# 1812598631/Amos-slam

Measured on AMD Instinct MI355X. Metric: front-end frames/sec (ORB extract+match+mask) at 640x480, higher is better.
Workload: dtype u8 (ORB, gate, matcher) + fp32 (mask network); 1 GPU; configs[2]: 640x480 L8 N1000 full front-end: YOLACT-R50 fp32 mask + ORB detect + gate + describe + match; lanes_per_gpu=2, frames_per_launch=64, width=640, height=480, n_features=1000, n_levels=8, ini_th_fast=20, min_th_fast=7, match=frame k vs k-1, N x N best-2, synthetic_stream_seed=stream = rank, frame k seeded 1000*rank+k (amos-slam_amd/synth.py), parallelism=frames sharded 1 ways, one process per GPU, no data-path collective

## Files before the change

amos-slam_amd/__init__.py:

```python
import ctypes as C
import os

import numpy as np

_HERE = os.path.dirname(os.path.abspath(__file__))
LIB_PATH = os.environ.get("AMOS_FRONTEND_LIB", os.path.join(_HERE, "csrc", "libamos_frontend.so"))

KP_DTYPE = np.dtype([("x", "<f4"), ("y", "<f4"), ("size", "<f4"), ("angle", "<f4"),
                     ("response", "<f4"), ("octave", "<i4"), ("class_id", "<i4")])
BEST2_DTYPE = np.dtype([("best_idx", "<i4"), ("best_dist", "<i4"), ("second_idx", "<i4"),
                        ("second_dist", "<i4")])

TH_HIGH, TH_LOW, HISTO_LENGTH = 100, 50, 30

EXPORTS = [
    "amos_last_error", "amos_device_count", "amos_current_device", "amos_build_variant", "amos_orb_tables_host", "amos_orb_geometry_probe", "amos_orb_create", "amos_orb_destroy", "amos_orb_tables",
    "amos_orb_level_sizes", "amos_orb_detect", "amos_orb_level_count", "amos_orb_level_keypoints",
    "amos_orb_set_level_keypoints", "amos_orb_level_layout", "amos_orb_fetch_levels", "amos_orb_store_levels", "amos_orb_gate", "amos_orb_closed_mask", "amos_orb_describe",
    "amos_orb_extract", "amos_orb_level_image", "amos_orb_pyramid_images", "amos_orb_blurred_image", "amos_orb_level_candidates",
    "amos_orb_extract_batch_device", "amos_orb_detect_batch_device", "amos_orb_gate_batch_device",
    "amos_orb_describe_batch_device", "amos_orb_extract_batch_device_color", "amos_frame_rgbd_glue_batch_device", "amos_frame_undistort_batch_device", "amos_frame_image_bounds", "amos_frame_grid_build_batch_device", "amos_match_window_best2_batch_device",
    "amos_orb_batch_results_device", "amos_orb_batch_fetch", "amos_orb_sync",
    "amos_orb_stream", "amos_orb_timing_enable", "amos_orb_timing_collect", "amos_match_create", "amos_match_destroy", "amos_match_sync", "amos_match_stream",
    "amos_match_distances", "amos_match_list_distances", "amos_match_list_best2", "amos_match_bruteforce_best2",
    "amos_match_bruteforce_best2_batch_device", "amos_match_set_bruteforce_kernel", "amos_slic_center_count", "amos_slic_create", "amos_slic_destroy", "amos_slic_stream",
    "amos_slic_run", "amos_slic_batch_device", "amos_cluster_kmeans_batch_device", "amos_cluster_kmeans", "amos_cluster_bgr2lab_batch_device", "amos_flow_check_device", "amos_flow_epipolar_device", "amos_flow_scene_flow_device", "amos_flow_fundamental_score_device", "amos_flow_pnp_score_device", "amos_lk_create", "amos_lk_destroy", "amos_lk_stream", "amos_lk_levels", "amos_lk_track_device", "amos_mask_pre_create", "amos_mask_pre_destroy", "amos_mask_pre_stream", "amos_mask_preprocess_batch_device", "amos_mask_bias_act_device", "amos_mask_bias_relu_maxpool_device", "amos_mask_stem_weight_floats", "amos_mask_stem_weights_device", "amos_mask_stem_device", "amos_mask_conv1x1_supported", "amos_mask_conv1x1_device", "amos_mask_conv_supported", "amos_mask_conv_device", "amos_mask_conv_workspace_bytes", "amos_mask_conv_ws_device", "amos_mask_conv_tile_mode", "amos_mask_conv_kernel_name", "amos_corners_create", "amos_corners_destroy", "amos_corners_stream", "amos_corners_good_features_device", "amos_corners_candidate_count", "amos_corners_subpix_device", "amos_fmat_create", "amos_fmat_destroy", "amos_fmat_stream", "amos_fmat_ransac_device", "amos_fmat_scene_flow_pair_device", "amos_fmat_ransac", "amos_mask_winograd_supported", "amos_mask_winograd_weight_floats", "amos_mask_winograd_weights_device", "amos_mask_winograd_conv_device", "amos_mask_winograd24_weight_floats", "amos_mask_winograd24_weights_device", "amos_mask_winograd24_conv_device", "amos_mask_winograd24_conv_layout_device", "amos_mask_winograd24_persistent_mode", "amos_mask_winograd24_narrow_mode", "amos_mask_bilinear_nhwc_device", "amos_mask_bilinear_nhwc_act_device", "amos_mask_bilinear_x2_mode", "amos_mask_nms_column_max_device", "amos_mask_class_scores_device", "amos_mask_person_mask_device", "amos_mask_head_outputs_device", "amos_mask_head_outputs_scores_device", "amos_mask_person_masks_scores_device", "amos_mask_topk_rows_device", "amos_mask_topk_rows_sparse_device", "amos_mask_post_workspace_bytes", "amos_mask_person_masks_device", "amos_orb_detect_color_with_mask_pre_batch_device",
]


class AmosError(RuntimeError):
    pass


class OrbParams(C.Structure):
    _fields_ = [("n_features", C.c_int32), ("scale_factor", C.c_float), ("n_levels", C.c_int32),
                ("ini_th_fast", C.c_int32), ("min_th_fast", C.c_int32)]


_lib = None


def lib():
    global _lib
    if _lib is None:
        if not os.path.exists(LIB_PATH):
            raise AmosError(f"{LIB_PATH} is missing: build it with `make -C amos-slam_amd/csrc` "
                            "(or __graft_entry__.build()); there is no CPU fallback")
        try:
            import torch
        except ImportError:
            pass
        L = C.CDLL(LIB_PATH)
        L.amos_last_error.restype = C.c_char_p
        L.amos_build_variant.restype = C.c_char_p
        variant = L.amos_build_variant().decode()
        if variant != "default" and os.environ.get("AMOS_ALLOW_EXPERIMENT_BUILD") != "1":
            raise AmosError(f"{LIB_PATH} is an experiment build ({variant}): its results are wrong; unset AMOS_FRONTEND_LIB "
                            "or set AMOS_ALLOW_EXPERIMENT_BUILD=1 for a timing run")
        L.amos_orb_stream.restype = C.c_void_p
# ... 427 lines not shown

def mask_winograd24_conv_layout(stream_ptr, x_ptr, u_ptr, bias_ptr, residual_ptr, y_ptr, batch, h, w, cin, cout, relu, in_blocked, out_blocked):
    _check(lib().amos_mask_winograd24_conv_layout_device(C.c_void_p(stream_ptr), C.c_void_p(x_ptr), C.c_void_p(u_ptr), C.c_void_p(bias_ptr),
                                                         C.c_void_p(residual_ptr), C.c_void_p(y_ptr), C.c_int(batch), C.c_int(h), C.c_int(w), C.c_int(cin),
                                                         C.c_int(cout), C.c_int(int(relu)), C.c_int(int(in_blocked)), C.c_int(int(out_blocked))),
           "amos_mask_winograd24_conv_layout_device")


def mask_winograd24_persistent_mode(mode=-2):
    return int(lib().amos_mask_winograd24_persistent_mode(C.c_int(mode)))


def mask_winograd24_narrow_mode(mode=-2):
    return int(lib().amos_mask_winograd24_narrow_mode(C.c_int(mode)))


def mask_conv_tile_mode(mode=-2):
    return int(lib().amos_mask_conv_tile_mode(C.c_int(mode)))


def mask_conv_kernel_name(batch, in_h, in_w, cin, cout, kh, kw, stride, pad):
    buf = C.create_string_buffer(96)
    _check(lib().amos_mask_conv_kernel_name(C.c_int(batch), C.c_int(in_h), C.c_int(in_w), C.c_int(cin), C.c_int(cout), C.c_int(kh), C.c_int(kw),
                                            C.c_int(stride), C.c_int(pad), buf, C.c_int(96)), "amos_mask_conv_kernel_name")
    return buf.value.decode()


def mask_conv(stream_ptr, x_ptr, w_ptr, bias_ptr, residual_ptr, y_ptr, batch, in_h, in_w, cin, cout, kh, kw, stride, pad, relu):
    _check(lib().amos_mask_conv_device(C.c_void_p(stream_ptr), C.c_void_p(x_ptr), C.c_void_p(w_ptr), C.c_void_p(bias_ptr), C.c_void_p(residual_ptr),
                                       C.c_void_p(y_ptr), C.c_int(batch), C.c_int(in_h), C.c_int(in_w), C.c_int(cin), C.c_int(cout), C.c_int(kh), C.c_int(kw),
                                       C.c_int(stride), C.c_int(pad), C.c_int(int(relu))), "amos_mask_conv_device")


def mask_conv_workspace_bytes(batch, in_h, in_w, cin, cout, kh, kw, stride, pad):
    fn = lib().amos_mask_conv_workspace_bytes
    fn.restype = C.c_size_t
    return int(fn(C.c_int(batch), C.c_int(in_h), C.c_int(in_w), C.c_int(cin), C.c_int(cout), C.c_int(kh), C.c_int(kw), C.c_int(stride), C.c_int(pad)))


def mask_conv_ws(stream_ptr, x_ptr, w_ptr, bias_ptr, residual_ptr, y_ptr, batch, in_h, in_w, cin, cout, kh, kw, stride, pad, relu, workspace_ptr, workspace_bytes):
    _check(lib().amos_mask_conv_ws_device(C.c_void_p(stream_ptr), C.c_void_p(x_ptr), C.c_void_p(w_ptr), C.c_void_p(bias_ptr), C.c_void_p(residual_ptr),
                                          C.c_void_p(y_ptr), C.c_int(batch), C.c_int(in_h), C.c_int(in_w), C.c_int(cin), C.c_int(cout), C.c_int(kh), C.c_int(kw),
                                          C.c_int(stride), C.c_int(pad), C.c_int(int(relu)), C.c_void_p(workspace_ptr), C.c_size_t(workspace_bytes)),
           "amos_mask_conv_ws_device")


def mask_bilinear_nhwc(stream_ptr, x_ptr, y_ptr, n, in_h, in_w, out_h, out_w, channels, scale_h, scale_w, relu=False):
    _check(lib().amos_mask_bilinear_nhwc_act_device(C.c_void_p(stream_ptr), C.c_void_p(x_ptr), C.c_void_p(y_ptr), C.c_int(n), C.c_int(in_h), C.c_int(in_w),
                                                    C.c_int(out_h), C.c_int(out_w), C.c_int(channels), C.c_float(scale_h), C.c_float(scale_w), C.c_int(int(relu))),
           "amos_mask_bilinear_nhwc_act_device")


def mask_class_scores(stream_ptr, conf_ptr, scores_ptr, batch, n_priors, n_classes_with_background, threshold):
    _check(lib().amos_mask_class_scores_device(C.c_void_p(stream_ptr), C.c_void_p(conf_ptr), C.c_void_p(scores_ptr), C.c_int(batch), C.c_int(n_priors),
                                               C.c_int(n_classes_with_background), C.c_float(threshold)), "amos_mask_class_scores_device")


def mask_person_mask(stream_ptr, masks_ptr, flags_ptr, out_ptr, batch, n_det, mask_h, mask_w, out_h, out_w):
    _check(lib().amos_mask_person_mask_device(C.c_void_p(stream_ptr), C.c_void_p(masks_ptr), C.c_void_p(flags_ptr), C.c_void_p(out_ptr), C.c_int(batch),
                                              C.c_int(n_det), C.c_int(mask_h), C.c_int(mask_w), C.c_int(out_h), C.c_int(out_w)), "amos_mask_person_mask_device")


def mask_head_outputs(stream_ptr, raw_ptr, bias_ptr, loc_ptr, conf_ptr, coef_ptr, batch, cells, channels_padded, anchors, n_classes_with_background, mask_dim,
                      n_priors_total, prior_offset):
    _check(lib().amos_mask_head_outputs_device(C.c_void_p(stream_ptr), C.c_void_p(raw_ptr), C.c_void_p(bias_ptr), C.c_void_p(loc_ptr), C.c_void_p(conf_ptr),
                                               C.c_void_p(coef_ptr), C.c_int(batch), C.c_int(cells), C.c_int(channels_padded), C.c_int(anchors),
# ... 262 lines not shown
```

amos-slam_amd/csrc/amos_conv1x1.hip:

```cpp
#include <hip/hip_runtime.h>
#include <stdint.h>
#include <stdio.h>
#include <stdlib.h>

#include <algorithm>

#include "../../include/amos_frontend.h"
#include "amos_common.h"

namespace amos {

constexpr int kGemmBK = 32;
constexpr int kGemmPitch = kGemmBK + 4;

typedef float f32x16 __attribute__((ext_vector_type(16)));

__device__ __attribute__((aligned(16))) const float g_conv_zeros[4] = {0.f, 0.f, 0.f, 0.f};

struct ConvGemmArgs {
    const float *x, *w, *bias, *res;
    float *y;
    int M, N, K;
    int outW, outHW, inW, inH;
    int stride, relu, mTiles, nTiles;
    int kh, kw, pad;
    int splits, stagesPerSplit;
    float *partial;
    unsigned *counters;
};

template <int WM, int WN, int TI, bool kTaps>
__global__ __launch_bounds__(256) __attribute__((amdgpu_waves_per_eu(1, 2))) void k_conv_gemm(const ConvGemmArgs a)
{
    constexpr int BM = 32 * TI * WM, BN = 64 * WN;
    constexpr int XP = BM / 32, WP = BN / 32;
    constexpr int kStage = (BM + BN) * kGemmPitch;
    static_assert(2 * kStage >= BM * BN, "the epilogue stages the output tile in the same LDS");
    __shared__ __align__(16) float smem[2 * kStage];
    float(*Xs)[kStage] = reinterpret_cast<float(*)[kStage]>(smem);
    float(*Ws)[kStage] = reinterpret_cast<float(*)[kStage]>(smem + BM * kGemmPitch);
    const int xcd = blockIdx.x & 7, seq = blockIdx.x >> 3;
    const int nt = a.splits > 1 ? (int)blockIdx.x % a.nTiles : seq % a.nTiles;
    const int mt = a.splits > 1 ? (int)blockIdx.x / a.nTiles : (seq / a.nTiles) * 8 + xcd;
    if (mt >= a.mTiles) return;
    const int t = threadIdx.x, lane = t & 63, wave = t >> 6;
    const int wm = wave / WN, wn = wave % WN;
    const int pc = t & 7, pr = t >> 3;
    const float *xsrc[XP];
    int iy0[XP], ix0[XP];
#pragma unroll
    for (int i = 0; i < XP; i++) {
        const int m = min(mt * BM + pr + 32 * i, a.M - 1);
        iy0[i] = ix0[i] = 0;
        if (!kTaps && a.stride == 1) {
            xsrc[i] = a.x + (size_t)m * a.K + 4 * pc;
        } else {
            const int b = m / a.outHW, rem = m - b * a.outHW, oy = rem / a.outW, ox = rem - oy * a.outW;
            iy0[i] = oy * a.stride - a.pad;
            ix0[i] = ox * a.stride - a.pad;
            xsrc[i] = a.x + (((ptrdiff_t)b * a.inH + iy0[i]) * a.inW + ix0[i]) * a.K + 4 * pc;
        }
    }
    const int kcPerTap = a.K / kGemmBK, wRow = a.K * a.kh * a.kw;
    const float *wsrc[WP];
#pragma unroll
    for (int j = 0; j < WP; j++) wsrc[j] = a.w + (size_t)(nt * BN + pr + 32 * j) * wRow + 4 * pc;
    static_assert(XP == 4 && (WP == 2 || WP == 4), "the staging registers below are named one by one");
    float4 x0, x1, x2, x3, w0, w1, w2 = {}, w3 = {};
    const int stagesAll = (a.K / kGemmBK) * a.kh * a.kw;
    const int sBegin = a.splits > 1 ? (int)blockIdx.y * a.stagesPerSplit : 0;
    const int sEnd = a.splits > 1 ? min(sBegin + a.stagesPerSplit, stagesAll) : stagesAll;
    int fKc = 0, fDy = 0, fDx = 0;
    if (kTaps && sBegin > 0) {
        const int kcPerTap0 = a.K / kGemmBK, tap = sBegin / kcPerTap0;
        fKc = sBegin - tap * kcPerTap0;
        fDy = tap / a.kw;
        fDx = tap - fDy * a.kw;
    }
    typedef float f32x4 __attribute__((ext_vector_type(4)));
    typedef const __attribute__((address_space(1))) f32x4 *GlobalF4;
// ... 60 lines not shown
    _Pragma("unroll") for (int q = 0; q < (n); q++) {                                     \
        __builtin_amdgcn_sched_group_barrier(0x008, 1, 0);                                \
        __builtin_amdgcn_sched_group_barrier(mask, 1, 0);                                 \
    }
    constexpr int kFragReads = TI + 2, kMfmas = 8 * TI;
#define AMOS_GEMM_STAGE(s, buf, kStash, kFetch, kNext)                                    \
    {                                                                                     \
        AMOS_GEMM_LDFRAG(fa1, fb1, buf, 1);                                               \
        AMOS_GEMM_MFMAS(fa0, fb0);                                                        \
        AMOS_GEMM_INTERLEAVE(0x100, kFragReads);                                          \
        __builtin_amdgcn_sched_group_barrier(0x008, kMfmas, 0);                           \
        __builtin_amdgcn_sched_barrier(0);                                                \
        AMOS_GEMM_LDFRAG(fa0, fb0, buf, 2);                                               \
        if (kStash) AMOS_GEMM_STASH((buf) ^ 1);                                           \
        AMOS_GEMM_MFMAS(fa1, fb1);                                                        \
        AMOS_GEMM_INTERLEAVE(0x100, kFragReads);                                          \
        AMOS_GEMM_INTERLEAVE(0x200, XP + WP);                                             \
        __builtin_amdgcn_sched_group_barrier(0x008, kMfmas, 0);                           \
        __builtin_amdgcn_sched_barrier(0);                                                \
        AMOS_GEMM_LDFRAG(fa1, fb1, buf, 3);                                               \
        if (kFetch) AMOS_GEMM_FETCH((s) + 2);                                             \
        AMOS_GEMM_MFMAS(fa0, fb0);                                                        \
        AMOS_GEMM_INTERLEAVE(0x100, kFragReads);                                          \
        AMOS_GEMM_INTERLEAVE(0x020, XP + WP);                                             \
        __builtin_amdgcn_sched_group_barrier(0x008, kMfmas, 0);                           \
        __builtin_amdgcn_sched_barrier(0);                                                \
        __syncthreads();                                                                  \
        if (kNext) AMOS_GEMM_LDFRAG(fa0, fb0, (buf) ^ 1, 0);                              \
        AMOS_GEMM_MFMAS(fa1, fb1);                                                        \
        AMOS_GEMM_INTERLEAVE(0x100, kFragReads);                                          \
        __builtin_amdgcn_sched_group_barrier(0x008, kMfmas, 0);                           \
        __builtin_amdgcn_sched_barrier(0);                                                \
    }
    f32x16 acc[TI][2];
#pragma unroll
    for (int i = 0; i < TI; i++)
#pragma unroll
        for (int j = 0; j < 2; j++)
#pragma unroll
            for (int r = 0; r < 16; r++) acc[i][j][r] = 0.f;
    const int xoff = (wm * 32 * TI + (lane & 31)) * kGemmPitch + 4 * (lane >> 5);
    const int woff = (wn * 64 + (lane & 31)) * kGemmPitch + 4 * (lane >> 5);
    const int stages = sEnd - sBegin;
    AMOS_GEMM_FETCH(sBegin);
    AMOS_GEMM_STASH(0);
    if (stages > 1) AMOS_GEMM_FETCH(sBegin + 1);
    __syncthreads();
    AMOS_GEMM_LDFRAG(fa0, fb0, 0, 0);
    int s = 0;
    for (; s + 2 < stages; s++) {
        const int buf = s & 1;
        AMOS_GEMM_STAGE(sBegin + s, buf, true, true, true);
    }
    if (s + 1 < stages) {
        const int buf = s & 1;
        AMOS_GEMM_STAGE(sBegin + s, buf, true, false, true);
        s++;
    }
    {
        const int buf = s & 1;
        AMOS_GEMM_STAGE(sBegin + s, buf, false, false, false);
    }
#undef AMOS_GEMM_FETCH
#undef AMOS_GEMM_TAPSRC
#undef AMOS_GEMM_STASH
#undef AMOS_GEMM_LDFRAG
#undef AMOS_GEMM_MFMAS
#undef AMOS_GEMM_INTERLEAVE
#undef AMOS_GEMM_STAGE
    __syncthreads();
#pragma unroll
    for (int i = 0; i < TI; i++)
#pragma unroll
        for (int j = 0; j < 2; j++)
#pragma unroll
            for (int r = 0; r < 16; r++)
                smem[(wm * 32 * TI + i * 32 + (r & 3) + 8 * (r >> 2) + 4 * (lane >> 5)) * BN + wn * 64 + j * 32 + (lane & 31)] = acc[i][j][r];
    __syncthreads();
    constexpr int kCols = BN / 4, kRowsPerPass = 256 / kCols, kPasses = BM / kRowsPerPass;
    const int oc = t % kCols, orow = t / kCols;
    const int n0 = nt * BN + 4 * oc;
    if (a.splits > 1) {
        __shared__ unsigned sArrived;
        const int tile = mt * a.nTiles + nt, nTilesAll = a.mTiles * a.nTiles;
        const unsigned xcc = __builtin_amdgcn_s_getreg((3 << 11) | 20) & 15u;
        const bool home = xcc == (blockIdx.x & 7u);
        float *mine = a.partial + ((size_t)blockIdx.y * nTilesAll + tile) * (BM * BN);
#pragma unroll
        for (int q = 0; q < kPasses; q++) {
            const int e = (q * kRowsPerPass + orow) * BN + 4 * oc;
            *reinterpret_cast<float4 *>(mine + e) = *reinterpret_cast<const float4 *>(&smem[e]);
        }
        if (home) asm volatile("s_waitcnt vmcnt(0)" ::: "memory");
        else __threadfence();
        __syncthreads();
        if (t == 0) sArrived = atomicAdd(&a.counters[tile], home ? 1u : 0x10001u);
        __syncthreads();
        const unsigned arrived = sArrived;
        if ((arrived & 0xffffu) != (unsigned)(a.splits - 1)) return;
        if (!home || (arrived >> 16) != 0) __threadfence();
#pragma unroll
        for (int q = 0; q < kPasses; q++) {
            const int e = (q * kRowsPerPass + orow) * BN + 4 * oc;
            float4 sum = {0.f, 0.f, 0.f, 0.f};
            for (int sp = 0; sp < a.splits; sp++) {
                typedef float f32x4v __attribute__((ext_vector_type(4)));
                const f32x4v v = *reinterpret_cast<const volatile f32x4v *>(a.partial + ((size_t)sp * nTilesAll + tile) * (BM * BN) + e);
                sum.x = sp ? sum.x + v.x : v.x; sum.y = sp ? sum.y + v.y : v.y; sum.z = sp ? sum.z + v.z : v.z; sum.w = sp ? sum.w + v.w : v.w;
            }
            *reinterpret_cast<float4 *>(&smem[e]) = sum;
        }
        if (t == 0) atomicExch(&a.counters[tile], 0u);
    }
    const float4 bv = a.bias ? *reinterpret_cast<const float4 *>(a.bias + n0) : float4{0.f, 0.f, 0.f, 0.f};
    constexpr int kBatch = 8;
#pragma unroll
    for (int p0 = 0; p0 < kPasses; p0 += kBatch) {
        float4 rv[kBatch];
#pragma unroll
        for (int q = 0; q < kBatch; q++) {
            const int m = mt * BM + (p0 + q) * kRowsPerPass + orow;
            rv[q] = (a.res && m < a.M) ? *reinterpret_cast<const float4 *>(a.res + (size_t)m * a.N + n0) : float4{0.f, 0.f, 0.f, 0.f};
        }
#pragma unroll
        for (int q = 0; q < kBatch; q++) {
            const int row = (p0 + q) * kRowsPerPass + orow, m = mt * BM + row;
            if (m >= a.M) continue;
            float4 v = *reinterpret_cast<const float4 *>(&smem[row * BN + 4 * oc]);
            v.x = (v.x + bv.x) + rv[q].x; v.y = (v.y + bv.y) + rv[q].y; v.z = (v.z + bv.z) + rv[q].z; v.w = (v.w + bv.w) + rv[q].w;
            if (a.relu) { v.x = fmaxf(v.x, 0.f); v.y = fmaxf(v.y, 0.f); v.z = fmaxf(v.z, 0.f); v.w = fmaxf(v.w, 0.f); }
            *reinterpret_cast<float4 *>(a.y + (size_t)m * a.N + n0) = v;
        }
    }
}

}

using namespace amos;

static int g_gemm_tile_mode = -2;

static int gemm_tile_mode()
{
    if (g_gemm_tile_mode == -2) {
        const char *env = getenv("AMOS_GEMM_NARROW");
        g_gemm_tile_mode = env && (env[0] == '0' || env[0] == '1') ? env[0] - '0' : -1;
    }
    return g_gemm_tile_mode;
}

static bool gemm_wide_tiles(long long M, int cout)
{
    const int mode = gemm_tile_mode();
    const long long wideGroups = ((M + 127) / 128) * (cout / 128);
    const bool narrow = mode >= 0 ? mode == 1 : wideGroups < 1024;
    return cout % 128 == 0 && !narrow;
}

extern "C" {

int amos_mask_conv_tile_mode(int mode)
{
    const int before = gemm_tile_mode();
// ... 44 lines not shown
    return (size_t)kSplitCounterBytes + (size_t)splits * tiles * 128 * (wide ? 128 : 64) * sizeof(float);
}

int amos_mask_conv_device(void *stream, const float *d_x, const float *d_w, const float *d_bias, const float *d_residual, float *d_y, int batch,
                          int in_h, int in_w, int cin, int cout, int kh, int kw, int stride, int pad, int relu)
{
    return amos_mask_conv_ws_device(stream, d_x, d_w, d_bias, d_residual, d_y, batch, in_h, in_w, cin, cout, kh, kw, stride, pad, relu, nullptr, 0);
}

int amos_mask_conv_ws_device(void *stream, const float *d_x, const float *d_w, const float *d_bias, const float *d_residual, float *d_y, int batch,
                             int in_h, int in_w, int cin, int cout, int kh, int kw, int stride, int pad, int relu, void *d_workspace, size_t workspace_bytes)
{
    if (!d_x || !d_w || !d_y || batch < 1 || in_h < 1 || in_w < 1 || amos_mask_conv_supported(cin, cout, kh, kw, stride, pad) != AMOS_OK ||
        in_h + 2 * pad < kh || in_w + 2 * pad < kw || ((uintptr_t)d_x | (uintptr_t)d_w | (uintptr_t)d_y | (uintptr_t)d_bias | (uintptr_t)d_residual) % 16 != 0) {
        set_error("amos_mask_conv_device: invalid argument (cin %% 32 == 0, cout %% 64 == 0, kernel <= 7 x 7, pad < kernel, stride 1..4, 16-byte aligned channels-last tensors)");
        return AMOS_ERR_INVALID;
    }
    const int oh = (in_h + 2 * pad - kh) / stride + 1, ow = (in_w + 2 * pad - kw) / stride + 1;
    const long long M = (long long)batch * oh * ow;
    if (M > 0x7fffffffLL / 4 || (long long)batch * in_h * in_w * cin > 0x7fffffffffLL) { set_error("amos_mask_conv_device: tensor too large"); return AMOS_ERR_INVALID; }
    ConvGemmArgs a;
    a.x = d_x; a.w = d_w; a.bias = d_bias; a.res = d_residual; a.y = d_y;
    a.M = (int)M; a.N = cout; a.K = cin;
    a.outW = ow; a.outHW = oh * ow; a.inW = in_w; a.inH = in_h;
    a.stride = stride; a.relu = relu; a.kh = kh; a.kw = kw; a.pad = pad;
    const bool wide = gemm_wide_tiles(M, cout), taps = kh * kw > 1 || pad > 0;
    const int BM = 128, BN = wide ? 128 : 64;
    a.mTiles = (int)((M + BM - 1) / BM);
    a.nTiles = cout / BN;
    a.splits = 1;
    a.stagesPerSplit = 0;
    a.partial = nullptr;
    a.counters = nullptr;
    if (d_workspace) {
        const int stages = (cin / kGemmBK) * kh * kw, splits = gemm_splits(M, cout, stages, wide);
        const size_t need = (size_t)kSplitCounterBytes + (size_t)splits * a.mTiles * a.nTiles * BM * BN * sizeof(float);
        if (splits > 1) {
            if (workspace_bytes < need || (uintptr_t)d_workspace % 16 != 0) { set_error("amos_mask_conv_ws_device: workspace of %zu bytes, %zu needed (16-byte aligned)", workspace_bytes, need); return AMOS_ERR_CAPACITY; }
            a.stagesPerSplit = (stages + splits - 1) / splits;
            a.splits = (stages + a.stagesPerSplit - 1) / a.stagesPerSplit;
            a.counters = (unsigned *)d_workspace;
            a.partial = (float *)((uint8_t *)d_workspace + kSplitCounterBytes);
        }
    }
    const dim3 grid(a.splits > 1 ? (unsigned)((a.mTiles * a.nTiles + 7) / 8 * 8) : (unsigned)(((a.mTiles + 7) / 8) * 8 * a.nTiles), (unsigned)a.splits), block(256);
    hipStream_t st = (hipStream_t)stream;
    if (wide && taps) hipLaunchKernelGGL((k_conv_gemm<2, 2, 2, true>), grid, block, 0, st, a);
    else if (wide) hipLaunchKernelGGL((k_conv_gemm<2, 2, 2, false>), grid, block, 0, st, a);
    else if (taps) hipLaunchKernelGGL((k_conv_gemm<4, 1, 1, true>), grid, block, 0, st, a);
    else hipLaunchKernelGGL((k_conv_gemm<4, 1, 1, false>), grid, block, 0, st, a);
    AMOS_HIP_CHECK(hipGetLastError());
    return AMOS_OK;
}

int amos_mask_conv1x1_supported(int cin, int cout, int stride) { return amos_mask_conv_supported(cin, cout, 1, 1, stride, 0); }

int amos_mask_conv1x1_device(void *stream, const float *d_x, const float *d_w, const float *d_bias, const float *d_residual, float *d_y, int batch,
                             int in_h, int in_w, int cin, int cout, int stride, int relu)
{
    return amos_mask_conv_device(stream, d_x, d_w, d_bias, d_residual, d_y, batch, in_h, in_w, cin, cout, 1, 1, stride, 0, relu);
}

}
```

amos-slam_amd/mask/net.py:

```python
import math
import os

import torch
import torch.nn as nn
import torch.nn.functional as F

NUM_CLASSES = 81
MASK_DIM = 32
FPN_FEATURES = 256
CONF_THRESH = 0.05
MAX_SIZE = 550
PRED_SCALES = (24, 48, 96, 192, 384)
ASPECT_RATIOS = (1.0, 0.5, 2.0)


def _gemm_conv(conv, x):
    k = conv.kernel_size
    if k[0] != k[1] or conv.padding[0] != conv.padding[1] or conv.dilation != (1, 1) or conv.groups != 1 or conv.stride[0] != conv.stride[1]:
        return False
    from .. import mask_conv_supported
    if not mask_conv_supported(conv.in_channels, conv.out_channels, k[0], k[1], conv.stride[0], conv.padding[0]):
        return False
    s = conv.stride[0]
    m = x.shape[0] * ((x.shape[2] + 2 * conv.padding[0] - k[0]) // s + 1) * ((x.shape[3] + 2 * conv.padding[1] - k[1]) // s + 1)
# ... 228 lines not shown
        oh, ow, sh, sw = geometry(h, w)
        y = Blocked(torch.empty((n, c // 8, oh, ow, 8), dtype=torch.float32, device=x.device), (n, c, oh, ow))
        from .. import mask_bilinear_nhwc
        mask_bilinear_nhwc(torch.cuda.current_stream(x.device).cuda_stream, x.data.data_ptr(), y.data.data_ptr(), n * (c // 8), h, w, oh, ow, 8, sh, sw, relu)
        return y
    if x.is_cuda and x.dtype == torch.float32 and x.shape[1] % 4 == 0 and x.is_contiguous(memory_format=torch.channels_last):
        n, c, h, w = x.shape
        oh, ow, sh, sw = geometry(h, w)
        y = torch.empty((n, c, oh, ow), dtype=torch.float32, device=x.device, memory_format=torch.channels_last)
        from .. import mask_bilinear_nhwc
        mask_bilinear_nhwc(torch.cuda.current_stream(x.device).cuda_stream, x.data_ptr(), y.data_ptr(), n, h, w, oh, ow, c, sh, sw, relu)
        return y
    if size is not None:
        y = F.interpolate(x, size=size, mode="bilinear", align_corners=False)
    else:
        y = F.interpolate(x, scale_factor=scale_factor, mode="bilinear", align_corners=False)
    return F.relu(y) if relu else y


def _fold(conv, bn):
    with torch.no_grad():
        scale = bn.weight.double() / torch.sqrt(bn.running_var.double() + bn.eps)
        w = (conv.weight.double() * scale.view(-1, 1, 1, 1)).to(conv.weight.dtype)
        b = bn.bias.double() - bn.running_mean.double() * scale
        if conv.bias is not None:
            b = b + conv.bias.double() * scale
        fused = nn.Conv2d(conv.in_channels, conv.out_channels, conv.kernel_size, conv.stride, conv.padding, conv.dilation, conv.groups, bias=True)
        fused = fused.to(device=conv.weight.device, dtype=conv.weight.dtype)
        fused.weight.copy_(w)
        fused.bias.copy_(b.to(conv.weight.dtype))
    return fused


class Bottleneck(nn.Module):
    expansion = 4

    def __init__(self, inplanes, planes, stride=1, project=False):
        super().__init__()
        self.conv1 = nn.Conv2d(inplanes, planes, 1, bias=False)
        self.bn1 = nn.BatchNorm2d(planes)
        self.conv2 = nn.Conv2d(planes, planes, 3, stride=stride, padding=1, bias=False)
        self.bn2 = nn.BatchNorm2d(planes)
        self.conv3 = nn.Conv2d(planes, planes * 4, 1, bias=False)
        self.bn3 = nn.BatchNorm2d(planes * 4)
        self.downsample = None
        if project:
            self.downsample = nn.Sequential(nn.Conv2d(inplanes, planes * 4, 1, stride=stride, bias=False),
                                            nn.BatchNorm2d(planes * 4))

    def forward(self, x):
        if self.conv1.bias is not None:
            y = conv_bias_act(self.conv1, x, True)
            y = conv_bias_act(self.conv2, y, True)
            identity = x if self.downsample is None else conv_bias_act(self.downsample[0], x, False)
            return conv_bias_act(self.conv3, y, True, residual=identity)
        y = F.relu(self.bn1(self.conv1(x)))
        y = F.relu(self.bn2(self.conv2(y)))
        y = self.bn3(self.conv3(y))
        return F.relu(y + (x if self.downsample is None else self.downsample(x)))

    def fold_batch_norms(self):
        for k in (1, 2, 3):
            setattr(self, f"conv{k}", _fold(getattr(self, f"conv{k}"), getattr(self, f"bn{k}")))
            setattr(self, f"bn{k}", nn.Identity())
        if self.downsample is not None:
            self.downsample = nn.Sequential(_fold(self.downsample[0], self.downsample[1]), nn.Identity())


class ResNet50Trunk(nn.Module):

    def __init__(self, blocks=(3, 4, 6, 3)):
        super().__init__()
        self.conv1 = nn.Conv2d(3, 64, 7, stride=2, padding=3, bias=False)
        self.bn1 = nn.BatchNorm2d(64)
        self.layers = nn.ModuleList()
        self.channels = []
        inplanes = 64
        for stage, (planes, n) in enumerate(zip((64, 128, 256, 512), blocks)):
            stride = 1 if stage == 0 else 2
            seq = [Bottleneck(inplanes, planes, stride, project=True)]
            inplanes = planes * 4
            seq += [Bottleneck(inplanes, planes) for _ in range(n - 1)]
            self.layers.append(nn.Sequential(*seq))
            self.channels.append(inplanes)

    def fold_batch_norms(self):
# ... 335 lines not shown
```

include/amos_frontend.h:

```cpp
#ifndef AMOS_FRONTEND_H
#define AMOS_FRONTEND_H

#include <stddef.h>
#include <stdint.h>

#ifdef __cplusplus
extern "C" {
#endif

#define AMOS_OK 0
#define AMOS_ERR_INVALID (-1)
#define AMOS_ERR_DEVICE (-2)
#define AMOS_ERR_CAPACITY (-3)
#define AMOS_ERR_STATE (-4)

#define AMOS_EDGE_THRESHOLD 19
#define AMOS_MAX_LEVELS 16
#define AMOS_FRAME_GRID_ROWS 48
#define AMOS_FRAME_GRID_COLS 64
#define AMOS_TH_HIGH 100
#define AMOS_TH_LOW 50
#define AMOS_HISTO_LENGTH 30

typedef struct amos_keypoint {
// ... 149 lines not shown

int amos_mask_pre_create(int device, void *stream, int width, int height, int max_batch, amos_mask_pre **out);
void amos_mask_pre_destroy(amos_mask_pre *p);
void *amos_mask_pre_stream(amos_mask_pre *p);
int amos_mask_preprocess_batch_device(amos_mask_pre *p, const uint8_t *d_bgr, int n_frames, float *d_out);

int amos_orb_detect_color_with_mask_pre_batch_device(amos_orb *h, amos_mask_pre *pre, const uint8_t *d_color,
                                                     size_t frame_stride, size_t row_stride, int width, int height,
                                                     int n_frames, int channels, int rgb_order, float *d_net_input);

int amos_mask_bias_act_device(void *stream, float *d_y, const float *d_bias, const float *d_residual, size_t n,
                              int channels, int relu);

int amos_mask_bias_relu_maxpool_device(void *stream, const float *d_x, const float *d_bias, float *d_y, int n, int in_h, int in_w,
                                       int channels);

int amos_mask_stem_weight_floats(void);
int amos_mask_stem_weights_device(void *stream, const float *d_w, long long stride_n, long long stride_c, long long stride_y, long long stride_x,
                                  float *d_packed);
int amos_mask_stem_device(void *stream, const float *d_x, long long stride_b, long long stride_c, long long stride_y, long long stride_x,
                          const float *d_packed, const float *d_bias, float *d_y, int batch, int height, int width);

int amos_mask_conv_supported(int cin, int cout, int kh, int kw, int stride, int pad);
int amos_mask_conv_device(void *stream, const float *d_x, const float *d_w, const float *d_bias, const float *d_residual,
                          float *d_y, int batch, int in_h, int in_w, int cin, int cout, int kh, int kw, int stride, int pad,
                          int relu);
size_t amos_mask_conv_workspace_bytes(int batch, int in_h, int in_w, int cin, int cout, int kh, int kw, int stride, int pad);
int amos_mask_conv_ws_device(void *stream, const float *d_x, const float *d_w, const float *d_bias, const float *d_residual, float *d_y,
                             int batch, int in_h, int in_w, int cin, int cout, int kh, int kw, int stride, int pad, int relu,
                             void *d_workspace, size_t workspace_bytes);
int amos_mask_conv_tile_mode(int mode);
int amos_mask_conv_kernel_name(int batch, int in_h, int in_w, int cin, int cout, int kh, int kw, int stride, int pad, char *name,
                               int name_len);
int amos_mask_conv1x1_supported(int cin, int cout, int stride);

int amos_mask_winograd_supported(int cin, int cout);
size_t amos_mask_winograd_weight_floats(int cin, int cout);
int amos_mask_winograd_weights_device(void *stream, const float *d_w, float *d_u, int cin, int cout);
int amos_mask_winograd_conv_device(void *stream, const float *d_x, const float *d_u, const float *d_bias, const float *d_residual,
                                   float *d_y, int batch, int h, int w, int cin, int cout, int relu);
size_t amos_mask_winograd24_weight_floats(int cin, int cout);
int amos_mask_winograd24_weights_device(void *stream, const float *d_w, float *d_u, int cin, int cout);
int amos_mask_winograd24_conv_device(void *stream, const float *d_x, const float *d_u, const float *d_bias, const float *d_residual,
                                     float *d_y, int batch, int h, int w, int cin, int cout, int relu);
int amos_mask_winograd24_conv_layout_device(void *stream, const float *d_x, const float *d_u, const float *d_bias, const float *d_residual,
                                            float *d_y, int batch, int h, int w, int cin, int cout, int relu, int in_blocked, int out_blocked);
int amos_mask_winograd24_persistent_mode(int mode);
int amos_mask_winograd24_narrow_mode(int mode);
int amos_mask_conv1x1_device(void *stream, const float *d_x, const float *d_w, const float *d_bias, const float *d_residual,
                             float *d_y, int batch, int in_h, int in_w, int cin, int cout, int stride, int relu);

int amos_mask_bilinear_nhwc_device(void *stream, const float *d_x, float *d_y, int n, int in_h, int in_w, int out_h,
                                   int out_w, int channels, float scale_h, float scale_w);

int amos_mask_bilinear_nhwc_act_device(void *stream, const float *d_x, float *d_y, int n, int in_h, int in_w, int out_h,
                                       int out_w, int channels, float scale_h, float scale_w, int relu);

int amos_mask_bilinear_x2_mode(int mode);

int amos_mask_nms_column_max_device(void *stream, const float *d_boxes, float *d_out, int n_lists, int k);

int amos_mask_class_scores_device(void *stream, const float *d_conf, float *d_scores, int batch, int n_priors,
                                  int n_classes_with_background, float threshold);

int amos_mask_person_mask_device(void *stream, const float *d_masks, const uint8_t *d_flags, uint8_t *d_out, int batch, int n_det,
                                 int mask_h, int mask_w, int out_h, int out_w);
// ... 110 lines not shown
```

Measured before the change: 1543 frames/s.

## Fuse bottleneck downsample 1x1 conv into conv3 GEMM as a two-phase kernel

```diff
diff --git a/amos-slam_amd/__init__.py b/amos-slam_amd/__init__.py
--- a/amos-slam_amd/__init__.py
+++ b/amos-slam_amd/__init__.py
@@ -24,7 +24,7 @@
     "amos_orb_stream", "amos_orb_timing_enable", "amos_orb_timing_collect", "amos_match_create", "amos_match_destroy", "amos_match_sync", "amos_match_stream",
     "amos_match_distances", "amos_match_list_distances", "amos_match_list_best2", "amos_match_bruteforce_best2",
     "amos_match_bruteforce_best2_batch_device", "amos_match_set_bruteforce_kernel", "amos_slic_center_count", "amos_slic_create", "amos_slic_destroy", "amos_slic_stream",
-    "amos_slic_run", "amos_slic_batch_device", "amos_cluster_kmeans_batch_device", "amos_cluster_kmeans", "amos_cluster_bgr2lab_batch_device", "amos_flow_check_device", "amos_flow_epipolar_device", "amos_flow_scene_flow_device", "amos_flow_fundamental_score_device", "amos_flow_pnp_score_device", "amos_lk_create", "amos_lk_destroy", "amos_lk_stream", "amos_lk_levels", "amos_lk_track_device", "amos_mask_pre_create", "amos_mask_pre_destroy", "amos_mask_pre_stream", "amos_mask_preprocess_batch_device", "amos_mask_bias_act_device", "amos_mask_bias_relu_maxpool_device", "amos_mask_stem_weight_floats", "amos_mask_stem_weights_device", "amos_mask_stem_device", "amos_mask_conv1x1_supported", "amos_mask_conv1x1_device", "amos_mask_conv_supported", "amos_mask_conv_device", "amos_mask_conv_workspace_bytes", "amos_mask_conv_ws_device", "amos_mask_conv_tile_mode", "amos_mask_conv_kernel_name", "amos_corners_create", "amos_corners_destroy", "amos_corners_stream", "amos_corners_good_features_device", "amos_corners_candidate_count", "amos_corners_subpix_device", "amos_fmat_create", "amos_fmat_destroy", "amos_fmat_stream", "amos_fmat_ransac_device", "amos_fmat_scene_flow_pair_device", "amos_fmat_ransac", "amos_mask_winograd_supported", "amos_mask_winograd_weight_floats", "amos_mask_winograd_weights_device", "amos_mask_winograd_conv_device", "amos_mask_winograd24_weight_floats", "amos_mask_winograd24_weights_device", "amos_mask_winograd24_conv_device", "amos_mask_winograd24_conv_layout_device", "amos_mask_winograd24_persistent_mode", "amos_mask_winograd24_narrow_mode", "amos_mask_bilinear_nhwc_device", "amos_mask_bilinear_nhwc_act_device", "amos_mask_bilinear_x2_mode", "amos_mask_nms_column_max_device", "amos_mask_class_scores_device", "amos_mask_person_mask_device", "amos_mask_head_outputs_device", "amos_mask_head_outputs_scores_device", "amos_mask_person_masks_scores_device", "amos_mask_topk_rows_device", "amos_mask_topk_rows_sparse_device", "amos_mask_post_workspace_bytes", "amos_mask_person_masks_device", "amos_orb_detect_color_with_mask_pre_batch_device",
+    "amos_slic_run", "amos_slic_batch_device", "amos_cluster_kmeans_batch_device", "amos_cluster_kmeans", "amos_cluster_bgr2lab_batch_device", "amos_flow_check_device", "amos_flow_epipolar_device", "amos_flow_scene_flow_device", "amos_flow_fundamental_score_device", "amos_flow_pnp_score_device", "amos_lk_create", "amos_lk_destroy", "amos_lk_stream", "amos_lk_levels", "amos_lk_track_device", "amos_mask_pre_create", "amos_mask_pre_destroy", "amos_mask_pre_stream", "amos_mask_preprocess_batch_device", "amos_mask_bias_act_device", "amos_mask_bias_relu_maxpool_device", "amos_mask_stem_weight_floats", "amos_mask_stem_weights_device", "amos_mask_stem_device", "amos_mask_conv1x1_supported", "amos_mask_conv1x1_device", "amos_mask_conv_supported", "amos_mask_conv_device", "amos_mask_conv_workspace_bytes", "amos_mask_conv_ws_device", "amos_mask_conv_tile_mode", "amos_mask_conv_kernel_name", "amos_mask_conv_chain_supported", "amos_mask_conv_chain_device", "amos_corners_create", "amos_corners_destroy", "amos_corners_stream", "amos_corners_good_features_device", "amos_corners_candidate_count", "amos_corners_subpix_device", "amos_fmat_create", "amos_fmat_destroy", "amos_fmat_stream", "amos_fmat_ransac_device", "amos_fmat_scene_flow_pair_device", "amos_fmat_ransac", "amos_mask_winograd_supported", "amos_mask_winograd_weight_floats", "amos_mask_winograd_weights_device", "amos_mask_winograd_conv_device", "amos_mask_winograd24_weight_floats", "amos_mask_winograd24_weights_device", "amos_mask_winograd24_conv_device", "amos_mask_winograd24_conv_layout_device", "amos_mask_winograd24_persistent_mode", "amos_mask_winograd24_narrow_mode", "amos_mask_bilinear_nhwc_device", "amos_mask_bilinear_nhwc_act_device", "amos_mask_bilinear_x2_mode", "amos_mask_nms_column_max_device", "amos_mask_class_scores_device", "amos_mask_person_mask_device", "amos_mask_head_outputs_device", "amos_mask_head_outputs_scores_device", "amos_mask_person_masks_scores_device", "amos_mask_topk_rows_device", "amos_mask_topk_rows_sparse_device", "amos_mask_post_workspace_bytes", "amos_mask_person_masks_device", "amos_orb_detect_color_with_mask_pre_batch_device",
 ]
 
 
@@ -518,6 +518,17 @@
                                        C.c_int(stride), C.c_int(pad), C.c_int(int(relu))), "amos_mask_conv_device")
 
 
+def mask_conv_chain_supported(batch, in_h, in_w, cin, planes, cout, stride):
+    return lib().amos_mask_conv_chain_supported(C.c_int(batch), C.c_int(in_h), C.c_int(in_w), C.c_int(cin), C.c_int(planes), C.c_int(cout),
+                                                C.c_int(stride)) == 0
+
+
+def mask_conv_chain(stream_ptr, x_ptr, wd_ptr, bd_ptr, yc_ptr, w3_ptr, b3_ptr, y_ptr, batch, in_h, in_w, cin, planes, cout, stride):
+    _check(lib().amos_mask_conv_chain_device(C.c_void_p(stream_ptr), C.c_void_p(x_ptr), C.c_void_p(wd_ptr), C.c_void_p(bd_ptr), C.c_void_p(yc_ptr),
+                                             C.c_void_p(w3_ptr), C.c_void_p(b3_ptr), C.c_void_p(y_ptr), C.c_int(batch), C.c_int(in_h), C.c_int(in_w),
+                                             C.c_int(cin), C.c_int(planes), C.c_int(cout), C.c_int(stride)), "amos_mask_conv_chain_device")
+
+
 def mask_conv_workspace_bytes(batch, in_h, in_w, cin, cout, kh, kw, stride, pad):
     fn = lib().amos_mask_conv_workspace_bytes
     fn.restype = C.c_size_t
diff --git a/amos-slam_amd/csrc/amos_conv1x1.hip b/amos-slam_amd/csrc/amos_conv1x1.hip
--- a/amos-slam_amd/csrc/amos_conv1x1.hip
+++ b/amos-slam_amd/csrc/amos_conv1x1.hip
@@ -27,11 +27,14 @@
     int splits, stagesPerSplit;
     float *partial;
     unsigned *counters;
+    const float *sx, *sw, *sbias;
+    int sK, sStride, sInW, sInH;
 };
 
-template <int WM, int WN, int TI, bool kTaps>
-__global__ __launch_bounds__(256) __attribute__((amdgpu_waves_per_eu(1, 2))) void k_conv_gemm(const ConvGemmArgs a)
-{
+template <int WM, int WN, int TI, bool kTaps, bool kShortcut = false>
+__global__ __launch_bounds__(256) __attribute__((amdgpu_waves_per_eu(1, 2))) void k_conv_gemm(const ConvGemmArgs args)
+{
+    static_assert(!(kShortcut && kTaps), "the shortcut form is a pair of 1 x 1 GEMMs");
     constexpr int BM = 32 * TI * WM, BN = 64 * WN;
     constexpr int XP = BM / 32, WP = BN / 32;
     constexpr int kStage = (BM + BN) * kGemmPitch;
@@ -40,12 +43,19 @@
     float(*Xs)[kStage] = reinterpret_cast<float(*)[kStage]>(smem);
     float(*Ws)[kStage] = reinterpret_cast<float(*)[kStage]>(smem + BM * kGemmPitch);
     const int xcd = blockIdx.x & 7, seq = blockIdx.x >> 3;
-    const int nt = a.splits > 1 ? (int)blockIdx.x % a.nTiles : seq % a.nTiles;
-    const int mt = a.splits > 1 ? (int)blockIdx.x / a.nTiles : (seq / a.nTiles) * 8 + xcd;
-    if (mt >= a.mTiles) return;
+    const int nt = args.splits > 1 ? (int)blockIdx.x % args.nTiles : seq % args.nTiles;
+    const int mt = args.splits > 1 ? (int)blockIdx.x / args.nTiles : (seq / args.nTiles) * 8 + xcd;
+    if (mt >= args.mTiles) return;
     const int t = threadIdx.x, lane = t & 63, wave = t >> 6;
     const int wm = wave / WN, wn = wave % WN;
     const int pc = t & 7, pr = t >> 3;
+    f32x16 acc[TI][2];
+    f32x16 dres[kShortcut ? TI : 1][2];
+    for (int phase = kShortcut ? 0 : 1; phase < 2; phase++) {
+    ConvGemmArgs a = args;
+    if (kShortcut && phase == 0) {
+        a.x = args.sx; a.w = args.sw; a.K = args.sK; a.stride = args.sStride; a.inW = args.sInW; a.inH = args.sInH;
+    }
     const float *xsrc[XP];
     int iy0[XP], ix0[XP];
 #pragma unroll
@@ -172,7 +182,6 @@
         __builtin_amdgcn_sched_group_barrier(0x008, kMfmas, 0);                           \
         __builtin_amdgcn_sched_barrier(0);                                                \
     }
-    f32x16 acc[TI][2];
 #pragma unroll
     for (int i = 0; i < TI; i++)
 #pragma unroll
@@ -208,7 +217,21 @@
 #undef AMOS_GEMM_MFMAS
 #undef AMOS_GEMM_INTERLEAVE
 #undef AMOS_GEMM_STAGE
+    if (kShortcut && phase == 0) {
+#pragma unroll
+        for (int j = 0; j < 2; j++) {
+            const float bd = args.sbias[nt * BN + wn * 64 + j * 32 + (lane & 31)];
+#pragma unroll
+            for (int i = 0; i < TI; i++)
+#pragma unroll
+                for (int r = 0; r < 16; r++) dres[i][j][r] = (acc[i][j][r] + bd) + 0.f;
+        }
+        __syncthreads();
+    }
+    }
+    const ConvGemmArgs &a = args;
     __syncthreads();
+    if constexpr (!kShortcut) {
 #pragma unroll
     for (int i = 0; i < TI; i++)
 #pragma unroll
@@ -216,11 +239,23 @@
 #pragma unroll
             for (int r = 0; r < 16; r++)
                 smem[(wm * 32 * TI + i * 32 + (r & 3) + 8 * (r >> 2) + 4 * (lane >> 5)) * BN + wn * 64 + j * 32 + (lane & 31)] = acc[i][j][r];
+    } else {
+#pragma unroll
+        for (int j = 0; j < 2; j++) {
+            const float b = a.bias[nt * BN + wn * 64 + j * 32 + (lane & 31)];
+#pragma unroll
+            for (int i = 0; i < TI; i++)
+#pragma unroll
+                for (int r = 0; r < 16; r++)
+                    smem[(wm * 32 * TI + i * 32 + (r & 3) + 8 * (r >> 2) + 4 * (lane >> 5)) * BN + wn * 64 + j * 32 + (lane & 31)] =
+                        fmaxf((acc[i][j][r] + b) + dres[i][j][r], 0.f);
+        }
+    }
     __syncthreads();
     constexpr int kCols = BN / 4, kRowsPerPass = 256 / kCols, kPasses = BM / kRowsPerPass;
     const int oc = t % kCols, orow = t / kCols;
     const int n0 = nt * BN + 4 * oc;
-    if (a.splits > 1) {
+    if (!kShortcut && a.splits > 1) {
         __shared__ unsigned sArrived;
         const int tile = mt * a.nTiles + nt, nTilesAll = a.mTiles * a.nTiles;
         const unsigned xcc = __builtin_amdgcn_s_getreg((3 << 11) | 20) & 15u;
@@ -267,8 +302,10 @@
             const int row = (p0 + q) * kRowsPerPass + orow, m = mt * BM + row;
             if (m >= a.M) continue;
             float4 v = *reinterpret_cast<const float4 *>(&smem[row * BN + 4 * oc]);
-            v.x = (v.x + bv.x) + rv[q].x; v.y = (v.y + bv.y) + rv[q].y; v.z = (v.z + bv.z) + rv[q].z; v.w = (v.w + bv.w) + rv[q].w;
-            if (a.relu) { v.x = fmaxf(v.x, 0.f); v.y = fmaxf(v.y, 0.f); v.z = fmaxf(v.z, 0.f); v.w = fmaxf(v.w, 0.f); }
+            if constexpr (!kShortcut) {
+                v.x = (v.x + bv.x) + rv[q].x; v.y = (v.y + bv.y) + rv[q].y; v.z = (v.z + bv.z) + rv[q].z; v.w = (v.w + bv.w) + rv[q].w;
+                if (a.relu) { v.x = fmaxf(v.x, 0.f); v.y = fmaxf(v.y, 0.f); v.z = fmaxf(v.z, 0.f); v.w = fmaxf(v.w, 0.f); }
+            }
             *reinterpret_cast<float4 *>(a.y + (size_t)m * a.N + n0) = v;
         }
     }
@@ -379,6 +416,8 @@
     a.stagesPerSplit = 0;
     a.partial = nullptr;
     a.counters = nullptr;
+    a.sx = a.sw = a.sbias = nullptr;
+    a.sK = a.sStride = a.sInW = a.sInH = 0;
     if (d_workspace) {
         const int stages = (cin / kGemmBK) * kh * kw, splits = gemm_splits(M, cout, stages, wide);
         const size_t need = (size_t)kSplitCounterBytes + (size_t)splits * a.mTiles * a.nTiles * BM * BN * sizeof(float);
@@ -400,6 +439,44 @@
     return AMOS_OK;
 }
 
+int amos_mask_conv_chain_supported(int batch, int in_h, int in_w, int cin, int planes, int cout, int stride)
+{
+    if (batch < 1 || in_h < 1 || in_w < 1 || amos_mask_conv_supported(cin, cout, 1, 1, stride, 0) != AMOS_OK || amos_mask_conv_supported(planes, cout, 1, 1, 1, 0) != AMOS_OK)
+        return AMOS_ERR_INVALID;
+    const long long M = (long long)batch * ((in_h - 1) / stride + 1) * ((in_w - 1) / stride + 1);
+    if (M > 0x7fffffffLL / 4 || (long long)batch * in_h * in_w * cin > 0x7fffffffffLL) return AMOS_ERR_INVALID;
+    return gemm_wide_tiles(M, cout) ? AMOS_OK : AMOS_ERR_INVALID;
+}
+
+int amos_mask_conv_chain_device(void *stream, const float *d_x, const float *d_wd, const float *d_bd, const float *d_yc, const float *d_w3, const float *d_b3,
+                                float *d_y, int batch, int in_h, int in_w, int cin, int planes, int cout, int stride)
+{
+    if (!d_x || !d_wd || !d_bd || !d_yc || !d_w3 || !d_b3 || !d_y || amos_mask_conv_chain_supported(batch, in_h, in_w, cin, planes, cout, stride) != AMOS_OK ||
+        ((uintptr_t)d_x | (uintptr_t)d_wd | (uintptr_t)d_yc | (uintptr_t)d_w3 | (uintptr_t)d_b3 | (uintptr_t)d_y) % 16 != 0) {
+        set_error("amos_mask_conv_chain_device: invalid argument (amos_mask_conv_chain_supported, both biases, 16-byte aligned channels-last tensors)");
+        return AMOS_ERR_INVALID;
+    }
+    const int oh = (in_h - 1) / stride + 1, ow = (in_w - 1) / stride + 1;
+    const long long M = (long long)batch * oh * ow;
+    ConvGemmArgs a;
+    a.x = d_yc; a.w = d_w3; a.bias = d_b3; a.res = nullptr; a.y = d_y;
+    a.M = (int)M; a.N = cout; a.K = planes;
+    a.outW = ow; a.outHW = oh * ow; a.inW = ow; a.inH = oh;
+    a.stride = 1; a.relu = 1; a.kh = a.kw = 1; a.pad = 0;
+    a.mTiles = (int)((M + 127) / 128);
+    a.nTiles = cout / 128;
+    a.splits = 1;
+    a.stagesPerSplit = 0;
+    a.partial = nullptr;
+    a.counters = nullptr;
+    a.sx = d_x; a.sw = d_wd; a.sbias = d_bd;
+    a.sK = cin; a.sStride = stride; a.sInW = in_w; a.sInH = in_h;
+    const dim3 grid((unsigned)(((a.mTiles + 7) / 8) * 8 * a.nTiles)), block(256);
+    hipLaunchKernelGGL((k_conv_gemm<2, 2, 2, false, true>), grid, block, 0, (hipStream_t)stream, a);
+    AMOS_HIP_CHECK(hipGetLastError());
+    return AMOS_OK;
+}
+
 int amos_mask_conv1x1_supported(int cin, int cout, int stride) { return amos_mask_conv_supported(cin, cout, 1, 1, stride, 0); }
 
 int amos_mask_conv1x1_device(void *stream, const float *d_x, const float *d_w, const float *d_bias, const float *d_residual, float *d_y, int batch,
diff --git a/amos-slam_amd/mask/net.py b/amos-slam_amd/mask/net.py
--- a/amos-slam_amd/mask/net.py
+++ b/amos-slam_amd/mask/net.py
@@ -284,6 +284,26 @@
     return fused
 
 
+def shortcut_fusion(block, x, y):
+    if os.environ.get("AMOS_MASK_BOTTLENECK_FUSION", "1") == "0" or os.environ.get("AMOS_MASK_CONV1X1", "auto") != "auto":
+        return False
+    if block.downsample is None or block.conv3.bias is None or block.downsample[0].bias is None:
+        return False
+    down, conv3 = block.downsample[0], block.conv3
+    if down.kernel_size != (1, 1) or down.padding != (0, 0) or down.stride[0] != down.stride[1] or conv3.kernel_size != (1, 1) or conv3.stride != (1, 1):
+        return False
+    if not (x.dtype == y.dtype == down.weight.dtype == conv3.weight.dtype == torch.float32) or x.device.type == "cpu" or torch.is_autocast_enabled():
+        return False
+    b, c, h, w = x.shape
+    s = down.stride[0]
+    if c != down.in_channels or tuple(y.shape) != (b, conv3.in_channels, (h - 1) // s + 1, (w - 1) // s + 1) or down.out_channels != conv3.out_channels:
+        return False
+    if not (_gemm_conv(down, x) and _gemm_conv(conv3, y)):
+        return False
+    from .. import mask_conv_chain_supported
+    return mask_conv_chain_supported(b, h, w, c, conv3.in_channels, conv3.out_channels, s)
+
+
 class Bottleneck(nn.Module):
     expansion = 4
 
@@ -304,6 +324,16 @@
         if self.conv1.bias is not None:
             y = conv_bias_act(self.conv1, x, True)
             y = conv_bias_act(self.conv2, y, True)
+            cl = torch.channels_last
+            if shortcut_fusion(self, x, y) and x.is_contiguous(memory_format=cl) and y.is_contiguous(memory_format=cl) and all(
+                    c.weight.is_contiguous() or c.weight.is_contiguous(memory_format=cl) for c in (self.downsample[0], self.conv3)):
+                from .. import mask_conv_chain
+                down, b, _, h, w = self.downsample[0], *x.shape
+                out = torch.empty((b, self.conv3.out_channels, y.shape[2], y.shape[3]), device=x.device, dtype=torch.float32, memory_format=cl)
+                mask_conv_chain(torch.cuda.current_stream(x.device).cuda_stream, x.data_ptr(), down.weight.data_ptr(), down.bias.data_ptr(), y.data_ptr(),
+                                self.conv3.weight.data_ptr(), self.conv3.bias.data_ptr(), out.data_ptr(), b, h, w, down.in_channels, self.conv3.in_channels,
+                                self.conv3.out_channels, down.stride[0])
+                return out
             identity = x if self.downsample is None else conv_bias_act(self.downsample[0], x, False)
             return conv_bias_act(self.conv3, y, True, residual=identity)
         y = F.relu(self.bn1(self.conv1(x)))
diff --git a/include/amos_frontend.h b/include/amos_frontend.h
--- a/include/amos_frontend.h
+++ b/include/amos_frontend.h
@@ -205,6 +205,9 @@
 int amos_mask_conv_tile_mode(int mode);
 int amos_mask_conv_kernel_name(int batch, int in_h, int in_w, int cin, int cout, int kh, int kw, int stride, int pad, char *name,
                                int name_len);
+int amos_mask_conv_chain_supported(int batch, int in_h, int in_w, int cin, int planes, int cout, int stride);
+int amos_mask_conv_chain_device(void *stream, const float *d_x, const float *d_wd, const float *d_bd, const float *d_yc, const float *d_w3,
+                                const float *d_b3, float *d_y, int batch, int in_h, int in_w, int cin, int planes, int cout, int stride);
 int amos_mask_conv1x1_supported(int cin, int cout, int stride);
 
 int amos_mask_winograd_supported(int cin, int cout);
```

Measured after the change: 1567 frames/s (median of 6 runs). 1.5% higher.
